# SeanChenxy/TDRN

Hardware: AMD Instinct MI355X
Metric: frames/sec/GPU @320x320 dualrefinedet_vggbn; box Linf vs CPU ref (higher is better)
Workload: dtype bf16; 1 GPU; dualrefinedet_vggbn 320x320 multihead, bf16, batch 32 per GPU, forward + Detect(top_k 200, conf 0.01, nms 0.45), synthetic VOC-shaped frames + synthetic weights; global_batch=32, parallelism=frame-sharded x1, no per-frame collective, launch=eager, resident_batches=4, steps_in_flight=2

## Files before the change

include/tdrn_hip.h:

```cpp
#ifndef TDRN_HIP_H
#define TDRN_HIP_H

#include <stddef.h>
#include <stdint.h>

#ifdef __cplusplus
extern "C" {
#endif

#define TDRN_API __attribute__((visibility("default")))

#define TDRN_OK 0
#define TDRN_E_ARG (-1)
#define TDRN_E_SHAPE (-2)
#define TDRN_E_WORKSPACE (-3)
#define TDRN_E_UNSUPPORTED (-4)
#define TDRN_E_PARAM (-5)
#define TDRN_E_STATE (-6)
#define TDRN_E_VALUE (-7)
#define TDRN_E_DEVICE (-8)

TDRN_API const char *tdrn_version(void);
TDRN_API const char *tdrn_error_string(int code);

// ... 161 lines not shown
#define TDRN_PLAN_ONE_STREAM    4
#define TDRN_PLAN_NO_DEFORM_TS  8
#define TDRN_PLAN_CHAIN         16
#define TDRN_PLAN_NO_CONV_PP    32
#define TDRN_PLAN_NO_PP_SK      64
#define TDRN_PLAN_NO_CONV_PATCH 128
#define TDRN_PLAN_DWPW          512
#define TDRN_PLAN_NO_PW1X1      1024
#define TDRN_PLAN_NO_DW_SLIDE   2048
#define TDRN_PLAN_DW_SLIDE_ALL  4096
#define TDRN_PLAN_NO_CONV_WS    8192
#define TDRN_PLAN_NO_YGEMM_V2  16384
#define TDRN_PLAN_NO_HEAD3X3   32768
#define TDRN_PLAN_TS_ONE_RANGE  65536
#define TDRN_PLAN_NO_PATCH_TAIL 131072
#define TDRN_PLAN_FAULT_HANDOFF 256

typedef struct tdrn_net tdrn_net;

TDRN_API int tdrn_net_create(const tdrn_net_config *cfg, tdrn_net **out);
TDRN_API void tdrn_net_destroy(tdrn_net *net);

TDRN_API int tdrn_net_param_count(const tdrn_net *net);
TDRN_API int tdrn_net_param_info(const tdrn_net *net, int index, const char **name,
                                 int64_t shape[4], int *ndim);
TDRN_API int tdrn_net_set_param(tdrn_net *net, const char *name, const float *data_host,
                                int64_t numel);

TDRN_API size_t tdrn_net_weight_bytes(const tdrn_net *net);
TDRN_API size_t tdrn_net_workspace_bytes(const tdrn_net *net, int batch);
// ... 72 lines not shown
```

tdrn_amd/_lib.py:

```python
import ctypes as C
import os

_HERE = os.path.dirname(os.path.abspath(__file__))
LIB_PATH = os.environ.get("TDRN_LIB_PATH") or os.path.join(_HERE, "lib", "libtdrn_hip.so")

F32, BF16, F16 = 0, 1, 2
DTYPES = {"fp32": F32, "f32": F32, "float32": F32, "bf16": BF16, "bfloat16": BF16, "fp16": F16,
          "f16": F16, "float16": F16, "half": F16}
DRN_VGGBN, DRN_MOBILENET, SSD4SCALE_MOBILE, REFINEDET_VGG, SSD4SCALE_VGG = range(5)

E_VALUE = -7


class TdrnError(RuntimeError):
    def __init__(self, code, what=""):
        self.code = code
        super().__init__("%s (tdrn error %d)%s" % (error_string(code), code,
                                                    (": " + what) if what else ""))


class NetConfig(C.Structure):
    _fields_ = [("model", C.c_int), ("size", C.c_int), ("num_classes", C.c_int),
                ("c7_channel", C.c_int), ("def_groups", C.c_int), ("bn", C.c_int),
                ("multihead", C.c_int), ("deform", C.c_int), ("test_phase", C.c_int),
                ("dtype", C.c_int), ("use_refine", C.c_int), ("plan_flags", C.c_int), ("reserved", C.c_int * 4)]


PLAN_NO_FUSE_FIRST, PLAN_NO_LATE_SIDE, PLAN_ONE_STREAM, PLAN_NO_DEFORM_TS, PLAN_CHAIN = 1, 2, 4, 8, 16
PLAN_NO_CONV_PP, PLAN_NO_PP_SK, PLAN_NO_CONV_PATCH, PLAN_FAULT_HANDOFF, PLAN_DWPW, PLAN_NO_PW1X1 = 32, 64, 128, 256, 512, 1024
PLAN_NO_DW_SLIDE, PLAN_DW_SLIDE_ALL, PLAN_NO_CONV_WS, PLAN_NO_YGEMM_V2, PLAN_NO_HEAD3X3, PLAN_TS_ONE_RANGE = 2048, 4096, 8192, 16384, 32768, 65536
PLAN_NO_PATCH_TAIL = 131072
E_DEVICE = -8


class NetIO(C.Structure):
    _fields_ = [("x", C.c_void_p), ("batch", C.c_int), ("arm_loc", C.c_void_p),
                ("odm_loc", C.c_void_p), ("conf", C.c_void_p), ("offsets", C.c_void_p * 4),
                ("ref_loc", C.c_void_p * 4), ("loc_maps", C.c_void_p * 4),
                ("reserved", C.c_void_p * 4)]


class KernelStat(C.Structure):
    _fields_ = [("name", C.c_char * 48), ("launches", C.c_int), ("flops", C.c_double),
                ("bytes", C.c_double), ("ms", C.c_double)]


# ... 166 lines not shown
```

tdrn_amd/csrc/conv3x3_patch.hip:

```cpp
#include <cstdio>
#include <cstdlib>
#include <type_traits>

#include "kernels.h"

#ifndef TDRN_PATCH_PRIO
#define TDRN_PATCH_PRIO 4
#endif
#ifndef TDRN_PATCH_ABLATE
#define TDRN_PATCH_ABLATE 0
#endif

namespace tdrn {

struct PatchParams {
    const char *in, *w, *zero;
    const float *bias;
    char *out, *out_pool;
    int B, H, W, Cin, Cout, Cs, Ktot;
    int relu;
    int tw, lgtw;
    int tiles_x, tiles_per_img;
    int m_tiles, n_tiles, items;
    int M;
    int tail_split;
    const float *fx, *fw, *fb;
    int fS, fCout;
    int ablate;
#ifdef TDRN_PATCH_STAMP
    unsigned *stamps;
#endif
#ifdef TDRN_PATCH_WGTIME
    unsigned long long *wgt;
#endif
};

#ifdef TDRN_PATCH_STAMP
#define STAMP_DECL unsigned long long st_t = __builtin_amdgcn_s_memtime(); unsigned st_acc[8] = {0, 0, 0, 0, 0, 0, 0, 0};
#define STAMP(k) do { const unsigned long long t_ = __builtin_amdgcn_s_memtime(); st_acc[k] += (unsigned)(t_ - st_t); st_t = t_; } while (0)
#define STAMP_FLUSH do { if (lane == 0) for (int k_ = 0; k_ < 8; ++k_) p.stamps[((size_t)blockIdx.x * 12 + wave) * 8 + k_] = st_acc[k_]; } while (0)
#else
#define STAMP_DECL
#define STAMP(k) do { } while (0)
// ... 76 lines not shown
    constexpr int RING = BN == 128 ? kRing : 3;
    constexpr int SROWS = (ES == 2 ? 16 : 8) / ((RING == 4 && BN == 128) ? 2 : 1);
    constexpr int SSTRIDE = BNH * ES + 16;
    constexpr int NPB = FUSE ? 1 : 2;
    constexpr int PSLOTS = FUSE ? ((TH + 2) * (TW + 2) + 7) / 8 : kPatchSlots;
    constexpr int PBYTES = PSLOTS * 1024;
    constexpr int OFF_W = NPB * PBYTES;
    constexpr int OFF_S = OFF_W + RING * WBYTES;
    constexpr int OFF_B = OFF_S + 8 * SROWS * SSTRIDE;
    constexpr int RAWR = TH + 4, RAWC = 36;
    constexpr int RAWN = 3 * RAWR * RAWC;
    constexpr int RAWP = (RAWN + 63) / 64, RAWJ = (RAWP + 3) / 4;
    constexpr int FTILES = ((TH + 2) * (TW + 2) + 31) / 32, FTJ = (FTILES + 3) / 4;
    constexpr int RAWB = ((RAWN + 63) / 64) * 256;
    constexpr int OFF_R = OFF_B + 1024;
    constexpr int LDS = FUSE ? OFF_R + 2 * RAWB + 256 : OFF_B + 1024;
    static_assert(LDS <= 160 * 1024, "LDS budget");
    __shared__ __attribute__((aligned(16))) char smem[LDS];

    const int lane = threadIdx.x & 63;
    const int wave = __builtin_amdgcn_readfirstlane(threadIdx.x >> 6);
    const int nchunks = p.Cin / CK;
#ifdef TDRN_PATCH_WGTIME
    if (threadIdx.x == 0) p.wgt[2 * blockIdx.x] = __builtin_amdgcn_s_memrealtime();
#endif

    const int xcd = blockIdx.x & 7, slot = blockIdx.x >> 3;
    const int per_xcd = (p.items + 7) >> 3, istride = ((int)gridDim.x + 7) >> 3;
    int avail = p.items - xcd * per_xcd;
    avail = avail < per_xcd ? avail : per_xcd;
    int n_full = avail > slot ? (avail - slot + istride - 1) / istride : 0;
    const int item0 = xcd * per_xcd + slot;
    [[maybe_unused]] int n_tail = 0, tail_enc = 0;
    constexpr bool TAILOK = BN == 128 && sizeof(DT) == 2 && !FUSE;
    if constexpr (TAILOK) {
        if (p.tail_split && avail > 0) {
            const int full = avail / istride, rem = avail - full * istride;
            if (full > 0 && rem > 0 && 2 * rem <= istride) {
                n_full = full;
                if (slot < 2 * rem) {
                    n_tail = 1;
                    tail_enc = 2 * (xcd * per_xcd + full * istride) + slot;
                }
            }
        }
    }
    const int n_it = n_full + n_tail;
    const int n_steps = n_it * nchunks * 9;
    auto item_mt = [&](int it) { return (it < n_full ? item0 + it * istride : tail_enc >> 1) / p.n_tiles; };
    auto item_c0 = [&](int it) {
        const int item = it < n_full ? item0 + it * istride : tail_enc >> 1;
        return (item % p.n_tiles) * BN + (it < n_full ? 0 : (tail_enc & 1) * 64);
    };
    const int RS = TW ? TW + 2 : p.W;

    if (wave >= 8) {
        if (TDRN_PATCH_PRIO == 4) __builtin_amdgcn_s_setprio(2);
        if (TDRN_PATCH_PRIO == 5) __builtin_amdgcn_s_setprio(3);
        const int lw = wave - 8;
        const int lrow = lane >> 3, pc = lane & 7;
        unsigned poff[kSlotsPerLoader];
        int pyx[kSlotsPerLoader];
        int plc[kSlotsPerLoader];
        {
#pragma unroll
            for (int j = 0; j < kSlotsPerLoader; ++j) {
                const int pr = (lw + 4 * j) * 8 + lrow;
                plc[j] = (pc ^ ((pr >> 1) & 7)) << 4;
// ... 131 lines not shown
#pragma unroll
                for (int j = 0; j < kSlotsPerLoader; ++j) {
                    const long long pix = j0 + pyx[j];
                    const bool ok = pyx[j] >= 0 && pix >= 0 && pix < p.M;
                    poff[j] = ok ? (unsigned)(pix * rowbytes + plc[j]) : 0xFFFFFFFFu;
                }
            }
        };
        unsigned woff[WL];
#pragma unroll
        for (int k = 0; k < WL; ++k) {
            const int n = (lw + 4 * k) * 8 + lrow;
            woff[k] = (unsigned)((size_t)n * p.Ktot * ES + ((pc ^ ((n >> 1) & 7)) << 4));
        }
        constexpr bool live = !(TDRN_PATCH_ABLATE & 1);
        int ws = 0, w_it = 0, w_cc = 0, w_tap = 0, wslot = 0;
        const char *wbase = p.w;
        unsigned wk = 0;
        int w_pieces = WL;
        auto weight_item = [&]() {
            wbase = p.w + (size_t)item_c0(w_it) * p.Ktot * ES;
            if constexpr (TAILOK) w_pieces = w_it < n_full ? WL : WL / 2;
        };
        constexpr bool wfixed = (TDRN_PATCH_ABLATE & 16) != 0, pfixed = (TDRN_PATCH_ABLATE & 32) != 0;
        auto load_weights = [&]() -> int {
            const int np = w_pieces;
            if (live) {
                char *dst = smem + OFF_W + wslot * WBYTES;
#pragma unroll
                for (int k = 0; k < WL; ++k)
                    if (!TAILOK || k < np) glds(wfixed ? p.w + (woff[k] & 0xffffu) : wbase + wk + woff[k], dst + (lw + 4 * k) * 1024);
            }
            ++ws;
            wslot = wslot == RING - 1 ? 0 : wslot + 1;
            wk += (unsigned)(p.Cin * ES);
            if (++w_tap == 9) {
                w_tap = 0;
                if (++w_cc == nchunks) {
                    w_cc = 0;
                    ++w_it;
                    if (w_it < n_it) weight_item();
                }
                wk = (unsigned)(w_cc * 128);
            }
            return np;
        };
        auto load_patch = [&](int j, unsigned ccoff, char *dstbuf) {
            if (!live || lw + 4 * j >= kPatchSlots || FUSE) return;
            const unsigned o = poff[j];
            glds(o == 0xFFFFFFFFu ? p.zero : (pfixed ? p.in + (o & 0xfffffu) : p.in + (size_t)o + ccoff), dstbuf + (lw + 4 * j) * 1024);
        };
        int p_it = 0, p_cc = 0, pbuf = 0;
        auto next_patch_chunk = [&]() {
            if (NPB == 2) pbuf ^= 1;
            if (++p_cc == nchunks) {
                p_cc = 0;
                ++p_it;
            }
        };

        if constexpr (FUSE) {
            if (n_it > 0) load_raw(item0, 0);
            asm volatile("s_waitcnt vmcnt(0) lgkmcnt(0)" ::: "memory");
            __builtin_amdgcn_s_barrier();
            if (n_it > 0) {
                int b_;
                tile_origin(item0, b_, f_y0, f_x0);
#pragma unroll
                for (int q = 0; q < FTJ; ++q)
                    if (lw + 4 * q < FTILES) first_conv_tile(lw + 4 * q, 0, smem);
            }
        }
        if (n_it > 0) {
            weight_item();
            if constexpr (!FUSE) {
                patch_table(item_mt(0));
#pragma unroll
                for (int j = 0; j < kSlotsPerLoader; ++j) load_patch(j, 0u, smem);
            }
#pragma unroll
            for (int k = 0; k < RING - 1; ++k)
                if (k < n_steps) load_weights();
            next_patch_chunk();
            if (lw == 0 && live)
                glds(lane < (n_full > 0 ? BN : 64) / 4 ? (const char *)(p.bias + item_c0(0)) + lane * 16 : p.zero, smem + OFF_B);
        }
        asm volatile("s_waitcnt vmcnt(0) lgkmcnt(0)" ::: "memory");
        __builtin_amdgcn_s_barrier();

        int tap = 0, c_it = 0, c_cc = 0, carried = 0;
        STAMP_DECL
        const int last_piece = lw + 4 * (kSlotsPerLoader - 1) < kPatchSlots ? 1 : 0;
        for (int g = 0; g < n_steps; ++g) {
            int issued = 0;
            if (ws < n_steps) issued = load_weights();
            if constexpr (FUSE) {
                if (tap == 0 && c_it + 1 < n_it) issued += load_raw(item0 + (c_it + 1) * istride, (c_it + 1) & 1);
            } else if (p_it < n_it && tap < 6) {
                char *dstbuf = smem + pbuf * PBYTES;
                const unsigned ccoff = (unsigned)(p_cc * 128);
                switch (tap) {
                    case 0:
                        patch_table(item_mt(p_it));
                        load_patch(0, ccoff, dstbuf); load_patch(1, ccoff, dstbuf); issued += 2; break;
                    case 1: load_patch(2, ccoff, dstbuf); load_patch(3, ccoff, dstbuf); issued += 2; break;
                    case 2: load_patch(4, ccoff, dstbuf); load_patch(5, ccoff, dstbuf); issued += 2; break;
                    case 3: load_patch(6, ccoff, dstbuf); load_patch(7, ccoff, dstbuf); issued += 2; break;
                    case 4: load_patch(8, ccoff, dstbuf); load_patch(9, ccoff, dstbuf); issued += 2; break;
                    default: load_patch(10, ccoff, dstbuf); issued += last_piece; break;
                }
            }
            if (lw == 0 && c_cc == nchunks - 1 && tap == 6 && c_it + 1 < n_it) {
                if (live) glds(lane < (c_it + 1 < n_full ? BN : 64) / 4 ? (const char *)(p.bias + item_c0(c_it + 1)) + lane * 16 : p.zero, smem + OFF_B);
                issued += 1;
            }
            STAMP(0);
            wait_vmcnt(live ? issued + (RING == 4 ? carried : 0) : 0);
            if constexpr (FUSE) asm volatile("s_waitcnt lgkmcnt(0)" ::: "memory");
            STAMP(1);
            carried = issued;
            __builtin_amdgcn_s_barrier();
            STAMP(2);
            if (++tap == 9) {
                tap = 0;
                next_patch_chunk();
                if (++c_cc == nchunks) {
                    if constexpr (FUSE) {
                        if (c_it + 1 < n_it) {
                            int b_;
                            tile_origin(item0 + (c_it + 1) * istride, b_, f_y0, f_x0);
#pragma unroll
                            for (int q = 0; q < FTJ; ++q)
                                if (lw + 4 * q < FTILES) first_conv_tile(lw + 4 * q, (c_it + 1) & 1, smem);
                            asm volatile("s_waitcnt lgkmcnt(0)" ::: "memory");
                            __builtin_amdgcn_s_barrier();
                        }
                    }
                    c_cc = 0;
                    ++c_it;
                }
            }
        }
        STAMP_FLUSH;
        return;
    }

    const int r32 = lane & 31, hh = lane >> 5;
    const int cw = wave % PXG;
    const int chalf = wave / PXG;
    char *stg = smem + OFF_S + wave * SROWS * SSTRIDE;
    f32x16 acc[WC][2];

    int base_i[2];
    unsigned tapmask[2] = {0x1FFu, 0x1FFu};
    unsigned need_mask = 0;
#pragma unroll
    for (int pt = 0; pt < 2; ++pt) {
        const int i = cw * 64 + pt * 32 + r32;
        base_i[pt] = TW ? (i >> LGTW) * RS + (i & (TW - 1)) : i;
    }
    const int wsw = (r32 >> 1) & 7;
    constexpr int CPR = BNH * ES / 16;
    constexpr int RPI = 64 / CPR;
    const int my_ch = lane % CPR, my_row = lane / CPR;
    constexpr bool compute = !(TDRN_PATCH_ABLATE & 2);

    int cur_mt = -1, n0 = 0;
    long long tile_pix0 = 0;
    int tile_row0 = 0, tile_x0 = 0;
    auto setup_item = [&](int it) {
        const int mt = item_mt(it);
        n0 = item_c0(it);
        if (mt == cur_mt) return;
        cur_mt = mt;
        if (TW) {
            const int b = mt / p.tiles_per_img, tt = mt - b * p.tiles_per_img;
            const int ty = tt / p.tiles_x, tx = tt - ty * p.tiles_x;
            tile_row0 = b * p.H + ty * TH;
            tile_x0 = tx * TW;
            tile_pix0 = (long long)tile_row0 * p.W + tile_x0;
            return;
        }
        tile_pix0 = (long long)mt * 256;
        need_mask = 0;
#pragma unroll
        for (int pt = 0; pt < 2; ++pt) {
            const long long m = tile_pix0 + cw * 64 + pt * 32 + r32;
// ... 230 lines not shown
    auto init_acc = [&](auto wcn_tag) {
        constexpr int WCN = decltype(wcn_tag)::value;
        const char *bsrc = smem + OFF_B;
#pragma unroll
        for (int ci = 0; ci < WCN; ++ci)
#pragma unroll
            for (int g = 0; g < 4; ++g) {
                const f32x4 bv = *(const f32x4 *)(bsrc + (chalf * (32 * WCN) + ci * 32 + 8 * g + 4 * hh) * 4);
#pragma unroll
                for (int pt = 0; pt < 2; ++pt)
#pragma unroll
                    for (int j = 0; j < 4; ++j) acc[ci][pt][4 * g + j] = bv[j];
            }
    };

    if constexpr (FUSE) __builtin_amdgcn_s_barrier();
    __builtin_amdgcn_s_barrier();
    if (TDRN_PATCH_PRIO == 2 && wave >= 4) __builtin_amdgcn_s_setprio(1);
    if (TDRN_PATCH_PRIO == 3) __builtin_amdgcn_s_setprio(1);
    typedef std::integral_constant<int, WC> full_t;
    typedef std::integral_constant<int, 1> half_t;
    if (n_it > 0) {
        setup_item(0);
        init_acc(full_t{});
        load_frags(full_t{}, wfA, pfA, 0);
    }
    int it = 0, cc = 0, tap = 0, tq = 0, delta = 0, wslot = 0, pbuf = 0;
    STAMP_DECL
    auto step = [&](auto wcn) {
        unsigned m0 = 0xFFFFFFFFu, m1 = 0xFFFFFFFFu;
        if constexpr (FLAT) {
            m0 = ((tapmask[0] >> tap) & 1u) ? 0xFFFFFFFFu : 0u;
            m1 = ((tapmask[1] >> tap) & 1u) ? 0xFFFFFFFFu : 0u;
        }
        if (TDRN_PATCH_PRIO == 0) __builtin_amdgcn_s_setprio(1);
        load_frags(wcn, wfB, pfB, 1);
        __builtin_amdgcn_sched_barrier(0);
        mma_frags(wcn, wfA, pfA, m0, m1);
        __builtin_amdgcn_sched_barrier(0);
        load_frags(wcn, wfA, pfA, 2);
        __builtin_amdgcn_sched_barrier(0);
        mma_frags(wcn, wfB, pfB, m0, m1);
// ... 21 lines not shown
        wsb = smem + OFF_W + wslot * WBYTES;
        psb = smem + (NPB == 2 ? pbuf : 0) * PBYTES;
#pragma unroll
        for (int pt = 0; pt < 2; ++pt) {
            prow[pt] = base_i[pt] + delta + tq;
            psw[pt] = (prow[pt] >> 1) & 7;
        }
        if (!(FUSE && item_done)) load_frags(wcn, wfA, pfA, 0);
        __builtin_amdgcn_sched_barrier(0);
        if (TDRN_PATCH_PRIO == 0) __builtin_amdgcn_s_setprio(1);
        mma_frags(wcn, wfB, pfB, m0, m1);
        if (TDRN_PATCH_PRIO == 0) __builtin_amdgcn_s_setprio(0);
        STAMP(2);
        if (item_done) {
            epilogue(wcn);
            ++it;
            if (it < n_it) {
                setup_item(it);
                if (TAILOK && it >= n_full) {
                    init_acc(half_t{});
                    load_frags(half_t{}, wfA, pfA, 0);
                } else {
                    init_acc(full_t{});
                }
                if constexpr (FUSE) {
                    __builtin_amdgcn_s_barrier();
                    load_frags(wcn, wfA, pfA, 0);
                }
            }
            STAMP(3);
        }
    };
    const int n_steps_full = n_full * nchunks * 9;
#pragma unroll 1
    for (int g = 0; g < n_steps_full; ++g) step(full_t{});
    if constexpr (TAILOK) {
#pragma unroll 1
        for (int g = n_steps_full; g < n_steps; ++g) step(half_t{});
    }
    STAMP_FLUSH;
#ifdef TDRN_PATCH_WGTIME
    if (threadIdx.x == 0) p.wgt[2 * blockIdx.x + 1] = __builtin_amdgcn_s_memrealtime();
#endif
}

int patch_conv_supported(const ConvArgs &a)
{
    if (a.kdisable & 4) return 0;
    if (a.kh != 3 || a.kw != 3 || a.stride != 1 || a.pad != 1 || a.dil != 1) return 0;
    if (a.phases != 1 || a.out_f32 || a.res) return 0;
    if (a.Ho != a.H || a.Wo != a.W) return 0;
    if (a.Npad % 64) return 0;
    if (a.o_rs != (long long)a.Wo * a.o_cs || a.o_bs != (long long)a.Ho * a.Wo * a.o_cs || a.o_base) return 0;
    if (!a.fuse_x && (long long)a.B * a.H * a.W * a.Cin * dtype_bytes(a.dtype) >= (1ll << 32)) return 0;
    if (a.W % 32 == 0 && a.H % 8 == 0) return 32;
    if (a.W % 16 == 0 && a.H % 16 == 0) return 16;
    if (2 * a.W + 2 + 256 <= kPatchSlots * 8) return -1;
    return 0;
}

template <typename DT, int BN> static int launch_patch_cfg(const PatchParams &p_in, hipStream_t s)
{
    PatchParams p = p_in;
    const int grid = p.items >= 256 ? 256 : ((p.items + 7) / 8) * 8;
#ifdef TDRN_PATCH_WGTIME
    static unsigned long long *wgt = nullptr;
    static long calls = 0, want = -1;
    if (!wgt) TDRN_HIP_TRY(hipMalloc((void **)&wgt, 256 * 2 * sizeof(unsigned long long)));
    if (want < 0) { const char *e = getenv("TDRN_WGTIME_CALL"); want = e ? atol(e) : 2000; }
    p.wgt = wgt;
    const bool report = calls >= want && calls < want + 18;
    ++calls;
    if (report) TDRN_HIP_TRY(hipMemsetAsync(wgt, 0, 256 * 2 * sizeof(unsigned long long), s));
    struct Report {
        bool on; hipStream_t s; int grid; const PatchParams &p; unsigned long long *d;
        ~Report() {
            if (!on) return;
            (void)hipStreamSynchronize(s);
            unsigned long long h[512];
            (void)hipMemcpy(h, d, sizeof(h), hipMemcpyDeviceToHost);
            unsigned long long t0 = ~0ull, t1 = 0;
            int n = 0;
            for (int i = 0; i < grid; ++i) if (h[2 * i]) { t0 = h[2 * i] < t0 ? h[2 * i] : t0; t1 = h[2 * i + 1] > t1 ? h[2 * i + 1] : t1; ++n; }
            double late = 0, busy = 0, worst = 0, e_min = 1e18; int n5 = 0, n20 = 0;
            for (int i = 0; i < grid; ++i) if (h[2 * i]) {
                const double d0 = (h[2 * i] - t0) * 0.01, b = (h[2 * i + 1] - h[2 * i]) * 0.01, e = (h[2 * i + 1] - t0) * 0.01;
                late += d0; busy += b; worst = d0 > worst ? d0 : worst; e_min = e < e_min ? e : e_min; n5 += d0 > 5; n20 += d0 > 20;
            }
            fprintf(stderr, "wgtime %dx%d Cin %d Cout %d items %d grid %d: span %.1f us, workgroup busy mean %.1f us, first end at %.1f us; start later than the first: mean %.1f us, max %.1f us, > 5 us: %d, > 20 us: %d of %d\n",
                    p.H, p.W, p.Cin, p.Cout, p.items, grid, (t1 - t0) * 0.01, busy / n, e_min, late / n, worst, n5, n20, n);
        }
    } rep{report, s, grid, p, wgt};
#endif
    if constexpr (BN == 64 && sizeof(DT) == 2) {
        if (p.fx) {
            if (p.tw != 32 || p.n_tiles != 1 || p.H % 16) return TDRN_E_UNSUPPORTED;
            hipLaunchKernelGGL((conv3x3_patch_kernel<DT, 64, 32, true>), dim3(grid), dim3(768), 0, s, p);
            return hip_status(hipGetLastError());
        }
    }
    if (p.fx) return TDRN_E_UNSUPPORTED;
    if (p.tw == 0) hipLaunchKernelGGL((conv3x3_patch_kernel<DT, BN, 0>), dim3(grid), dim3(768), 0, s, p);
    else if (p.tw == 32) hipLaunchKernelGGL((conv3x3_patch_kernel<DT, BN, 32>), dim3(grid), dim3(768), 0, s, p);
    else hipLaunchKernelGGL((conv3x3_patch_kernel<DT, BN, 16>), dim3(grid), dim3(768), 0, s, p);
    return hip_status(hipGetLastError());
// ... 25 lines not shown
        p.tiles_per_img = p.tiles_x * (a.H / ((a.fuse_x ? 512 : 256) / p.tw));
        p.m_tiles = a.B * p.tiles_per_img;
    } else {
        p.tiles_x = 0; p.tiles_per_img = 0;
        p.m_tiles = cdiv(p.M, 256);
    }
    int BN = a.Npad % 128 == 0 ? 128 : 64;
    if (BN == 128 && p.m_tiles * (a.Npad / 128) < 160) BN = 64;
    p.n_tiles = a.Npad / BN;
    p.items = p.m_tiles * p.n_tiles;
    static int ablate = -1;
    if (ablate < 0) ablate = dev_ablate_env("TDRN_CONV_ABLATE");
    p.ablate = ablate;
    p.fx = a.fuse_x; p.fw = a.fuse_w; p.fb = a.fuse_b; p.fS = a.H; p.fCout = a.fuse_cout;
    p.tail_split = !(a.kdisable & 1024);
    if (p.items <= 0) return TDRN_OK;
#ifdef TDRN_PATCH_STAMP
    static unsigned *stamps = nullptr;
    if (!stamps) TDRN_HIP_TRY(hipMalloc((void **)&stamps, 256 * 12 * 8 * sizeof(unsigned)));
    TDRN_HIP_TRY(hipMemsetAsync(stamps, 0, 256 * 12 * 8 * sizeof(unsigned), s));
    p.stamps = stamps;
    struct Report {
        const PatchParams &p; hipStream_t s; int BN, nchunks;
        ~Report()
        {
            static unsigned host[256 * 12 * 8];
            (void)hipStreamSynchronize(s);
            (void)hipMemcpy(host, p.stamps, sizeof(host), hipMemcpyDeviceToHost);
            double c[4] = {0, 0, 0, 0}, l[3] = {0, 0, 0};
            int nc = 0, nl = 0;
// ... 28 lines not shown
```

tdrn_amd/csrc/kernels.h:

```cpp
#pragma once
#include <cmath>

#include "common.h"

namespace tdrn {

constexpr size_t kZeroPageBytes = 256;

int allow_big_lds(const void *kernel);

struct ConvArgs {
    const void *in = nullptr, *w = nullptr, *res = nullptr, *zero_page = nullptr;
    const float *bias = nullptr;
    void *out = nullptr;
    int B = 0, H = 0, W = 0, Cin = 0;
    int Ho = 0, Wo = 0, Cout = 0, Npad = 0;
    int kh = 1, kw = 1, stride = 1, pad = 0, dil = 1;
    int relu = 0, out_f32 = 0, phases = 1;
    int splitk = 1;
    void *partial = nullptr;
    long long o_bs = 0, o_rs = 0, o_cs = 0, o_base = 0, o_pr = 0, o_pc = 0;
    int dtype = TDRN_BF16;
    const float *fuse_x = nullptr, *fuse_w = nullptr, *fuse_b = nullptr;
    int fuse_cout = 0;
    const unsigned char *fuse_x8 = nullptr;
    float fuse_mean[3] = {0.f, 0.f, 0.f};
    void *sk_ws = nullptr;
    bool sk_flags_zero = false;
    int kdisable = 0;
    unsigned *status = nullptr;
    int fault_handoff = 0;
};
int launch_conv(const ConvArgs &a, hipStream_t s);
struct ChainLayer { ConvArgs a; int dep[2] = {-1, -1}; };
int conv_chain_supported(const ConvArgs &a);
int conv_chain_max_layers();
size_t conv_chain_ctr_bytes();
int launch_conv_chain(const ChainLayer *layers, int n, unsigned *ctr, hipStream_t s, unsigned *status = nullptr);
int conv_splitk_choice(const ConvArgs &a);
size_t conv_splitk_bytes(const ConvArgs &a, int splits);
int head3x3_supported(const ConvArgs &a);
int launch_head3x3(const ConvArgs &a, hipStream_t s);
int patch_conv_supported(const ConvArgs &a);
// ... 142 lines not shown
```

tdrn_amd/csrc/net.hip:

```cpp
#include <algorithm>
#include <cmath>
#include <cstdlib>
#include <cstring>
#include <map>
#include <string>
#include <mutex>
#include <vector>

#include "kernels.h"

namespace tdrn {

unsigned short host_f32_to_bf16(float f)
{
    uint32_t u;
    memcpy(&u, &f, 4);
    if ((u & 0x7fffffffu) > 0x7f800000u) return (unsigned short)((u >> 16) | 0x40);
    return (unsigned short)((u + 0x7fffu + ((u >> 16) & 1u)) >> 16);
}
unsigned short host_f32_to_f16(float f)
{
    _Float16 h = (_Float16)f;
    unsigned short r;
    memcpy(&r, &h, 2);
// ... 106 lines not shown
    std::vector<ParamSpec> params;
    std::map<std::string, size_t> param_index;
    std::map<std::string, std::vector<float>> staged;
    std::vector<Op> ops;
    size_t ws_per_sample = 0, blob_bytes = kZeroPageBytes;
    size_t ws_fixed = 0;
    int P = 0, fm[4] = {0, 0, 0, 0}, scale_off[5] = {0, 0, 0, 0, 0};
    bool weights_ready = false;
    int profile = 0;
    std::vector<hipEvent_t> ev;
    std::vector<int> ev_stat;
    std::vector<int> ev_op;
    tdrn_kernel_stat stats[ST_COUNT];
    int last_batch = 0;
    static constexpr int kLanes = 4;
    static constexpr size_t kTailCtl = 256;
    size_t splitk_off[kLanes] = {0, 0, 0, 0};
    int cur_lane = 0;
    int t_late = -1;
    std::vector<int> chain_ops;
    size_t chain_partial_off = 0;
    bool pp_sk_planned = false;
    int fuse_first = -1;
    int x_t = -1;
    bool late_side = true;
    bool use_lanes = true, lanes_ready = false;
    bool y_tap_major = true;
    int plan_error = TDRN_OK;
    const void *offs_ws = nullptr;
    int offs_batch = 0, offs_key_batch = 0;
    int dev = -1;
// ... 454 lines not shown
            conv(src[s], "arm_conf." + ss, true, "", nc3, 3, 1, 1, 1, 0, -1, OUT_CONF, s);
            loc_maps_out(s);
        }
        if (cfg.test_phase) softmax_op();
        return TDRN_OK;
    }

    int build()
    {
        es = dtype_bytes(cfg.dtype);
        kdisable = ((cfg.plan_flags & TDRN_PLAN_NO_CONV_PP) ? 1 : 0) | ((cfg.plan_flags & TDRN_PLAN_NO_PP_SK) ? 2 : 0) |
                   ((cfg.plan_flags & TDRN_PLAN_NO_CONV_PATCH) ? 4 : 0) | ((cfg.plan_flags & TDRN_PLAN_NO_PW1X1) ? 8 : 0) |
                   ((cfg.plan_flags & TDRN_PLAN_NO_DW_SLIDE) ? 16 : 0) | ((cfg.plan_flags & TDRN_PLAN_DW_SLIDE_ALL) ? 32 : 0) |
                   ((cfg.plan_flags & TDRN_PLAN_NO_CONV_WS) ? 64 : 0) | ((cfg.plan_flags & TDRN_PLAN_NO_YGEMM_V2) ? 128 : 0) |
                   ((cfg.plan_flags & TDRN_PLAN_NO_HEAD3X3) ? 256 : 0) | ((cfg.plan_flags & TDRN_PLAN_TS_ONE_RANGE) ? 512 : 0) |
                   ((cfg.plan_flags & TDRN_PLAN_NO_PATCH_TAIL) ? 1024 : 0);
        fault_handoff = (cfg.plan_flags & TDRN_PLAN_FAULT_HANDOFF) ? 1 : 0;
        if (cfg.size < 128 || cfg.size > 1280 || cfg.size % 64 != 0) return TDRN_E_ARG;
        if (cfg.num_classes < 2 || cfg.num_classes > 21 * 4) return TDRN_E_ARG;
        if (cfg.dtype < 0 || cfg.dtype > 2) return TDRN_E_ARG;
        if (cfg.def_groups < 1) return TDRN_E_ARG;
        int rc;
        switch (cfg.model) {
            case TDRN_DRN_VGGBN: rc = build_drn_vgg(); break;
            case TDRN_DRN_MOBILENET: rc = build_drn_mobilenet(); break;
            case TDRN_SSD4SCALE_MOBILE: rc = build_ssd4scale(true); break;
            case TDRN_SSD4SCALE_VGG: rc = build_ssd4scale(false); break;
            case TDRN_REFINEDET_VGG: rc = build_refinedet_vgg(); break;
            default: return TDRN_E_UNSUPPORTED;
        }
        if (rc != TDRN_OK) return rc;
// ... 153 lines not shown
                DwPwArgs a;
                a.B = 1; a.H = ti.H; a.W = ti.W; a.Cin = c.Cin; a.Cout = c.Cout; a.Npad = c.Npad; a.Cs = tensors[c.out].Cpad;
                a.stride = d.stride; a.dtype = cfg.dtype;
                if (ti.Cpad != c.Cin || !dwpw_supported(a)) continue;
                d.fused_dw = 1; c.fused_dw = 1;
                d.stat = ST_DWPW;
                d.flops += c.flops;
                d.bytes = (double)ti.H * ti.W * ti.Cpad * es + (double)ti.H * ti.W * tensors[c.out].Cpad * es;
                c.flops = 0; c.bytes = 0;
            }
        ws_fixed = 0;
        pp_sk_planned = false;
        if (cfg.dtype != TDRN_F32)
            for (const Op &o : ops)
                if (o.kind == OP_CONV && o.stat == ST_CONV3 && o.lane == 0 && o.Cin >= 256 && o.Npad % 256 == 0) pp_sk_planned = true;
        if (pp_sk_planned || !chain_ops.empty()) ws_fixed = kTailCtl + (pp_sk_planned ? align_up(conv_pp_sk_bytes(), 256) : 1024);
        use_lanes = !(cfg.plan_flags & TDRN_PLAN_ONE_STREAM);
        y_tap_major = true;
        for (const Op &d : ops)
            if (d.kind == OP_DEFORM && d.y_t >= 0 && !ygemm_supported(d.Cin, d.y_cols, cfg.dtype)) y_tap_major = false;
        tensor_lane.assign(tensors.size(), 0);
        tensor_shared.assign(tensors.size(), 0);
        for (const Op &o : ops) {
            if (o.out >= 0) tensor_lane[o.out] = o.lane;
            if (o.pool_t >= 0) tensor_lane[o.pool_t] = o.lane;
        }
        for (const Op &o : ops)
            for (int t : {o.in, o.res, o.off_t})
                if (t >= 0 && tensor_lane[t] != o.lane) tensor_shared[t] = 1;
        return TDRN_OK;
    }
// ... 271 lines not shown
                    if ((ops[k].n_branches == 2 || (ops[k].G >= 2 && ops[k].G % 2 == 0)) && ops[k].y_t < 0 && !dsplit) dsplit = &ops[k];
                    if (k == 0 || ops[k - 1].kind != OP_DEFORM) ++n_deform_groups;
                }
            if (dsplit && n_deform_groups == 1) {
                float *locbase0 = dsplit->out_kind == OUT_ARM_LOC ? io->arm_loc : io->odm_loc;
                TDRN_HIP_TRY(hipStreamWaitEvent(side[0], ev_fork, 0));
                lane_used[1] = true;
                TDRN_HIP_TRY(hipMemsetAsync(locbase0, 0, (size_t)B * P * 4 * sizeof(float), side[0]));
                TDRN_HIP_TRY(hipMemsetAsync(io->conf, 0, (size_t)B * P * C * sizeof(float), side[0]));
                TDRN_HIP_TRY(hipEventRecord(ev_zero, side[0]));
                zeroed_early = true;
            }
        }
        bool skz_pending = false;
        char *const tail = (char *)ws + ws_per_sample * (size_t)B;
        if (ws_fixed) {
            if (lanes) {
                if (!lane_used[1]) {
                    TDRN_HIP_TRY(hipStreamWaitEvent(side[0], ev_fork, 0));
                    lane_used[1] = true;
                }
                TDRN_HIP_TRY(hipMemsetAsync(tail, 0, kTailCtl + 1024, side[0]));
                TDRN_HIP_TRY(hipEventRecord(ev_skz, side[0]));
                skz_pending = true;
            } else {
                TDRN_HIP_TRY(hipMemsetAsync(tail, 0, kTailCtl + 1024, s0));
            }
        }
        auto conv_args = [&](const Op &o, ConvArgs &a) {
            const Tensor &ti = tensors[o.in];
            a.in = tptr(ws, o.in, B); a.w = wb + o.w_off; a.bias = (const float *)(wb + o.b_off); a.zero_page = wb;
            a.B = B; a.H = ti.H; a.W = ti.W; a.Cin = o.Cin; a.Ho = o.hw >> 16; a.Wo = o.hw & 0xffff;
            a.Cout = o.Cout; a.Npad = o.Npad; a.kh = a.kw = o.k; a.stride = o.stride; a.pad = o.pad; a.dil = o.dil;
            a.relu = o.relu; a.phases = o.phases; a.dtype = cfg.dtype;
            a.kdisable = kdisable; a.status = status; a.fault_handoff = fault_handoff;
            if (o.out_kind == OUT_TENSOR) {
                const Tensor &to = tensors[o.out];
                a.out = tptr(ws, o.out, B);
                if (o.res >= 0) a.res = tptr(ws, o.res, B);
                a.o_cs = to.Cpad;
                if (o.phases == 4) {
                    a.o_bs = (long long)to.H * to.W * to.Cpad; a.o_rs = 2ll * to.W * to.Cpad; a.o_cs = 2ll * to.Cpad;
                    a.o_pr = (long long)to.W * to.Cpad; a.o_pc = to.Cpad;
                } else {
                    a.o_bs = (long long)to.H * to.W * to.Cpad; a.o_rs = (long long)to.W * to.Cpad;
                }
            } else {
                const int per = o.out_kind == OUT_CONF ? 3 * C : 12;
                const int per_prior = o.out_kind == OUT_CONF ? C : 4;
                float *base = o.out_kind == OUT_ARM_LOC ? io->arm_loc : (o.out_kind == OUT_ODM_LOC ? io->odm_loc : io->conf);
// ... 82 lines not shown
                        }
                        if (skz_pending) {
                            TDRN_HIP_TRY(hipStreamWaitEvent(s0, ev_skz, 0));
                            skz_pending = false;
                        }
                        rc = launch_conv_chain(cl, n, (unsigned *)tail, s, status);
                        if (rc == TDRN_OK && lanes)
                            for (int k = 1; k < n; ++k) {
                                const int t = ops[chain_ops[k]].out;
                                if (t >= 0 && tensor_shared[t]) TDRN_HIP_TRY(hipEventRecord(tensor_ev[t], s));
                            }
                        break;
                    }
                    ConvArgs a;
                    conv_args(o, a);
                    if (o.lane == 0 && pp_sk_planned) {
                        a.sk_ws = tail + kTailCtl;
                        a.sk_flags_zero = true;
                        if (skz_pending && pp_conv_supported(a)) {
                            TDRN_HIP_TRY(hipStreamWaitEvent(s0, ev_skz, 0));
                            skz_pending = false;
                        }
                    }
                    if ((int)oi == fuse_first) {
                        a.fuse_w = (const float *)(wb + ops[0].w_off); a.fuse_b = (const float *)(wb + ops[0].b_off);
                        a.fuse_cout = ops[0].Cout;
                        if (!xin && o.pool_t >= 0) {
                            a.fuse_x8 = u8->planes; a.fuse_mean[0] = u8->mean[0]; a.fuse_mean[1] = u8->mean[1]; a.fuse_mean[2] = u8->mean[2];
                            a.out = nullptr;
                            rc = ws_conv_supported(a) ? launch_conv3x3_ws(a, tptr(ws, o.pool_t, B), s) : TDRN_E_UNSUPPORTED;
// ... 509 lines not shown
```

Baseline: 12510 frames/s.

## Replace static item dealing in patch conv with per-XCD atomic work claiming

The patch 3x3 conv kernel now has a loader wave claim work units dynamically through a per-XCD global atomic counter, instead of each workgroup taking a fixed strided set of items. The claimed unit, which can be a full tile or a half tail unit, is passed to the compute waves through a two-slot LDS mailbox. The last workgroup to finish resets the counters, and the host reserves per-lane claim slots in the workspace tail and waits on the zeroing event before first use. This is meant to even out load imbalance when workgroups start late, at the cost of atomic latency, an extra mailbox handshake in the pipeline, and new cross-stream ordering requirements.

```diff
diff --git a/include/tdrn_hip.h b/include/tdrn_hip.h
--- a/include/tdrn_hip.h
+++ b/include/tdrn_hip.h
@@ -199,6 +199,7 @@
 #define TDRN_PLAN_NO_HEAD3X3   32768
 #define TDRN_PLAN_TS_ONE_RANGE  65536
 #define TDRN_PLAN_NO_PATCH_TAIL 131072
+#define TDRN_PLAN_NO_PATCH_CLAIM 262144
 #define TDRN_PLAN_FAULT_HANDOFF 256
 
 typedef struct tdrn_net tdrn_net;
diff --git a/tdrn_amd/_lib.py b/tdrn_amd/_lib.py
--- a/tdrn_amd/_lib.py
+++ b/tdrn_amd/_lib.py
@@ -29,7 +29,7 @@
 PLAN_NO_FUSE_FIRST, PLAN_NO_LATE_SIDE, PLAN_ONE_STREAM, PLAN_NO_DEFORM_TS, PLAN_CHAIN = 1, 2, 4, 8, 16
 PLAN_NO_CONV_PP, PLAN_NO_PP_SK, PLAN_NO_CONV_PATCH, PLAN_FAULT_HANDOFF, PLAN_DWPW, PLAN_NO_PW1X1 = 32, 64, 128, 256, 512, 1024
 PLAN_NO_DW_SLIDE, PLAN_DW_SLIDE_ALL, PLAN_NO_CONV_WS, PLAN_NO_YGEMM_V2, PLAN_NO_HEAD3X3, PLAN_TS_ONE_RANGE = 2048, 4096, 8192, 16384, 32768, 65536
-PLAN_NO_PATCH_TAIL = 131072
+PLAN_NO_PATCH_TAIL, PLAN_NO_PATCH_CLAIM = 131072, 262144
 E_DEVICE = -8
 
 
diff --git a/tdrn_amd/csrc/conv3x3_patch.hip b/tdrn_amd/csrc/conv3x3_patch.hip
--- a/tdrn_amd/csrc/conv3x3_patch.hip
+++ b/tdrn_amd/csrc/conv3x3_patch.hip
@@ -27,6 +27,7 @@
     const float *fx, *fw, *fb;
     int fS, fCout;
     int ablate;
+    unsigned *claim;
 #ifdef TDRN_PATCH_STAMP
     unsigned *stamps;
 #endif
@@ -133,7 +134,8 @@
     constexpr int FTILES = ((TH + 2) * (TW + 2) + 31) / 32, FTJ = (FTILES + 3) / 4;
     constexpr int RAWB = ((RAWN + 63) / 64) * 256;
     constexpr int OFF_R = OFF_B + 1024;
-    constexpr int LDS = FUSE ? OFF_R + 2 * RAWB + 256 : OFF_B + 1024;
+    constexpr int OFF_M = FUSE ? OFF_R + 2 * RAWB + 256 : OFF_B + 1024;
+    constexpr int LDS = OFF_M + 16;
     static_assert(LDS <= 160 * 1024, "LDS budget");
     __shared__ __attribute__((aligned(16))) char smem[LDS];
 
@@ -141,36 +143,17 @@
     const int wave = __builtin_amdgcn_readfirstlane(threadIdx.x >> 6);
     const int nchunks = p.Cin / CK;
 #ifdef TDRN_PATCH_WGTIME
-    if (threadIdx.x == 0) p.wgt[2 * blockIdx.x] = __builtin_amdgcn_s_memrealtime();
+    if (threadIdx.x == 0) p.wgt[3 * blockIdx.x] = __builtin_amdgcn_s_memrealtime();
 #endif
 
     const int xcd = blockIdx.x & 7, slot = blockIdx.x >> 3;
     const int per_xcd = (p.items + 7) >> 3, istride = ((int)gridDim.x + 7) >> 3;
-    int avail = p.items - xcd * per_xcd;
-    avail = avail < per_xcd ? avail : per_xcd;
-    int n_full = avail > slot ? (avail - slot + istride - 1) / istride : 0;
-    const int item0 = xcd * per_xcd + slot;
-    [[maybe_unused]] int n_tail = 0, tail_enc = 0;
+    typedef volatile __attribute__((address_space(3))) int lds_int;
+    lds_int *const mbox = (lds_int *)(smem + OFF_M);
     constexpr bool TAILOK = BN == 128 && sizeof(DT) == 2 && !FUSE;
-    if constexpr (TAILOK) {
-        if (p.tail_split && avail > 0) {
-            const int full = avail / istride, rem = avail - full * istride;
-            if (full > 0 && rem > 0 && 2 * rem <= istride) {
-                n_full = full;
-                if (slot < 2 * rem) {
-                    n_tail = 1;
-                    tail_enc = 2 * (xcd * per_xcd + full * istride) + slot;
-                }
-            }
-        }
-    }
-    const int n_it = n_full + n_tail;
-    const int n_steps = n_it * nchunks * 9;
-    auto item_mt = [&](int it) { return (it < n_full ? item0 + it * istride : tail_enc >> 1) / p.n_tiles; };
-    auto item_c0 = [&](int it) {
-        const int item = it < n_full ? item0 + it * istride : tail_enc >> 1;
-        return (item % p.n_tiles) * BN + (it < n_full ? 0 : (tail_enc & 1) * 64);
-    };
+    auto unit_mt = [&](int u) { return (u >> 2) / p.n_tiles; };
+    auto unit_half = [&](int u) { return TAILOK && (u & 2) != 0; };
+    auto unit_c0 = [&](int u) { return ((u >> 2) % p.n_tiles) * BN + (unit_half(u) ? (u & 1) * 64 : 0); };
     const int RS = TW ? TW + 2 : p.W;
 
     if (wave >= 8) {
@@ -332,13 +315,50 @@
             woff[k] = (unsigned)((size_t)n * p.Ktot * ES + ((pc ^ ((n >> 1) & 7)) << 4));
         }
         constexpr bool live = !(TDRN_PATCH_ABLATE & 1);
-        int ws = 0, w_it = 0, w_cc = 0, w_tap = 0, wslot = 0;
+        int n_whole = p.items - xcd * per_xcd;
+        n_whole = n_whole < per_xcd ? n_whole : per_xcd;
+        n_whole = n_whole > 0 ? n_whole : 0;
+        int n_units = n_whole;
+        if constexpr (TAILOK) {
+            if (p.tail_split) {
+                const int full = n_whole / istride, rem = n_whole - full * istride;
+                if (full > 0 && rem > 0 && 2 * rem <= istride) {
+                    n_whole = full * istride;
+                    n_units = n_whole + 2 * rem;
+                }
+            }
+        }
+        auto unit_of = [&](int k) -> int {
+            const int h = k - n_whole, base = xcd * per_xcd;
+            return (unsigned)k >= (unsigned)n_units ? -1 : (h < 0 ? (base + k) << 2 : (((base + n_whole + (h >> 1)) << 2) | 2 | (h & 1)));
+        };
+        int k_pend = 0, k_dealt = slot - istride;
+        auto claim_issue = [&]() -> int {
+            if (p.claim) {
+                if (lane == 0) k_pend = (int)__hip_atomic_fetch_add(p.claim + xcd, 1u, __ATOMIC_RELAXED, __HIP_MEMORY_SCOPE_AGENT);
+                return 1;
+            }
+            k_dealt += istride;
+            return 0;
+        };
+        auto claim_publish = [&](int m) {
+            if (p.claim) {
+                if (lane == 0) mbox[m & 1] = unit_of(k_pend);
+            } else if (lane == 0) {
+                mbox[m & 1] = unit_of(k_dealt);
+            }
+        };
+        int w_cc = 0, w_tap = 0, wslot = 0;
+        bool w_live = false;
         const char *wbase = p.w;
         unsigned wk = 0;
         int w_pieces = WL;
-        auto weight_item = [&]() {
-            wbase = p.w + (size_t)item_c0(w_it) * p.Ktot * ES;
-            if constexpr (TAILOK) w_pieces = w_it < n_full ? WL : WL / 2;
+        int u_p = -1;
+        auto weight_item = [&](int u) {
+            w_live = u >= 0;
+            if (!w_live) return;
+            wbase = p.w + (size_t)unit_c0(u) * p.Ktot * ES;
+            if constexpr (TAILOK) w_pieces = unit_half(u) ? WL / 2 : WL;
         };
         constexpr bool wfixed = (TDRN_PATCH_ABLATE & 16) != 0, pfixed = (TDRN_PATCH_ABLATE & 32) != 0;
         auto load_weights = [&]() -> int {
@@ -349,15 +369,13 @@
                 for (int k = 0; k < WL; ++k)
                     if (!TAILOK || k < np) glds(wfixed ? p.w + (woff[k] & 0xffffu) : wbase + wk + woff[k], dst + (lw + 4 * k) * 1024);
             }
-            ++ws;
             wslot = wslot == RING - 1 ? 0 : wslot + 1;
             wk += (unsigned)(p.Cin * ES);
             if (++w_tap == 9) {
                 w_tap = 0;
                 if (++w_cc == nchunks) {
                     w_cc = 0;
-                    ++w_it;
-                    if (w_it < n_it) weight_item();
+                    weight_item(u_p);
                 }
                 wk = (unsigned)(w_cc * 128);
             }
@@ -377,49 +395,63 @@
             }
         };
 
+        if (lw == 0) {
+            claim_issue();
+            claim_publish(0);
+            if (nchunks == 1) {
+                claim_issue();
+                claim_publish(1);
+            }
+        }
+        asm volatile("s_waitcnt vmcnt(0) lgkmcnt(0)" ::: "memory");
+        __builtin_amdgcn_s_barrier();
+        int u_c = __builtin_amdgcn_readfirstlane(mbox[0]);
+        u_p = u_c;
         if constexpr (FUSE) {
-            if (n_it > 0) load_raw(item0, 0);
+            if (u_c >= 0) load_raw(u_c >> 2, 0);
             asm volatile("s_waitcnt vmcnt(0) lgkmcnt(0)" ::: "memory");
             __builtin_amdgcn_s_barrier();
-            if (n_it > 0) {
+            if (u_c >= 0) {
                 int b_;
-                tile_origin(item0, b_, f_y0, f_x0);
+                tile_origin(u_c >> 2, b_, f_y0, f_x0);
 #pragma unroll
                 for (int q = 0; q < FTJ; ++q)
                     if (lw + 4 * q < FTILES) first_conv_tile(lw + 4 * q, 0, smem);
             }
         }
-        if (n_it > 0) {
-            weight_item();
+        if (u_c >= 0) {
+            weight_item(u_c);
             if constexpr (!FUSE) {
-                patch_table(item_mt(0));
+                patch_table(unit_mt(u_c));
 #pragma unroll
                 for (int j = 0; j < kSlotsPerLoader; ++j) load_patch(j, 0u, smem);
             }
 #pragma unroll
-            for (int k = 0; k < RING - 1; ++k)
-                if (k < n_steps) load_weights();
+            for (int k = 0; k < RING - 1; ++k) load_weights();
             next_patch_chunk();
             if (lw == 0 && live)
-                glds(lane < (n_full > 0 ? BN : 64) / 4 ? (const char *)(p.bias + item_c0(0)) + lane * 16 : p.zero, smem + OFF_B);
+                glds(lane < (unit_half(u_c) ? 64 : BN) / 4 ? (const char *)(p.bias + unit_c0(u_c)) + lane * 16 : p.zero, smem + OFF_B);
         }
         asm volatile("s_waitcnt vmcnt(0) lgkmcnt(0)" ::: "memory");
         __builtin_amdgcn_s_barrier();
 
-        int tap = 0, c_it = 0, c_cc = 0, carried = 0;
+        int tap = 0, c_cc = 0, carried = 0;
+        [[maybe_unused]] int c_it = 0;
         STAMP_DECL
         const int last_piece = lw + 4 * (kSlotsPerLoader - 1) < kPatchSlots ? 1 : 0;
-        for (int g = 0; g < n_steps; ++g) {
+        while (u_c >= 0) {
             int issued = 0;
-            if (ws < n_steps) issued = load_weights();
+            if (tap == 0 && p_cc == 0) u_p = __builtin_amdgcn_readfirstlane(mbox[p_it & 1]);
+            if (lw == 0 && tap == 3 && p_cc == nchunks - 1 && u_p >= 0) claim_publish(p_it + 1);
+            if (w_live) issued = load_weights();
             if constexpr (FUSE) {
-                if (tap == 0 && c_it + 1 < n_it) issued += load_raw(item0 + (c_it + 1) * istride, (c_it + 1) & 1);
-            } else if (p_it < n_it && tap < 6) {
+                if (tap == 0 && c_cc == nchunks - 1 && u_p >= 0) issued += load_raw(u_p >> 2, (c_it + 1) & 1);
+            } else if (u_p >= 0 && tap < 6) {
                 char *dstbuf = smem + pbuf * PBYTES;
                 const unsigned ccoff = (unsigned)(p_cc * 128);
                 switch (tap) {
                     case 0:
-                        patch_table(item_mt(p_it));
+                        patch_table(unit_mt(u_p));
                         load_patch(0, ccoff, dstbuf); load_patch(1, ccoff, dstbuf); issued += 2; break;
                     case 1: load_patch(2, ccoff, dstbuf); load_patch(3, ccoff, dstbuf); issued += 2; break;
                     case 2: load_patch(4, ccoff, dstbuf); load_patch(5, ccoff, dstbuf); issued += 2; break;
@@ -428,13 +460,14 @@
                     default: load_patch(10, ccoff, dstbuf); issued += last_piece; break;
                 }
             }
-            if (lw == 0 && c_cc == nchunks - 1 && tap == 6 && c_it + 1 < n_it) {
-                if (live) glds(lane < (c_it + 1 < n_full ? BN : 64) / 4 ? (const char *)(p.bias + item_c0(c_it + 1)) + lane * 16 : p.zero, smem + OFF_B);
+            if (lw == 0 && c_cc == nchunks - 1 && tap == 6 && u_p >= 0) {
+                if (live) glds(lane < (unit_half(u_p) ? 64 : BN) / 4 ? (const char *)(p.bias + unit_c0(u_p)) + lane * 16 : p.zero, smem + OFF_B);
                 issued += 1;
             }
+            if (lw == 0 && tap == 1 && p_cc == nchunks - 1 && u_p >= 0) issued += claim_issue();
             STAMP(0);
             wait_vmcnt(live ? issued + (RING == 4 ? carried : 0) : 0);
-            if constexpr (FUSE) asm volatile("s_waitcnt lgkmcnt(0)" ::: "memory");
+            if (FUSE || (lw == 0 && tap == 3)) asm volatile("s_waitcnt lgkmcnt(0)" ::: "memory");
             STAMP(1);
             carried = issued;
             __builtin_amdgcn_s_barrier();
@@ -444,9 +477,9 @@
                 next_patch_chunk();
                 if (++c_cc == nchunks) {
                     if constexpr (FUSE) {
-                        if (c_it + 1 < n_it) {
+                        if (u_p >= 0) {
                             int b_;
-                            tile_origin(item0 + (c_it + 1) * istride, b_, f_y0, f_x0);
+                            tile_origin(u_p >> 2, b_, f_y0, f_x0);
 #pragma unroll
                             for (int q = 0; q < FTJ; ++q)
                                 if (lw + 4 * q < FTILES) first_conv_tile(lw + 4 * q, (c_it + 1) & 1, smem);
@@ -456,10 +489,16 @@
                     }
                     c_cc = 0;
                     ++c_it;
+                    u_c = u_p;
                 }
             }
         }
         STAMP_FLUSH;
+        if (lw == 0 && lane == 0 && p.claim) {
+            const unsigned done = __hip_atomic_fetch_add(p.claim + 8, 1u, __ATOMIC_RELAXED, __HIP_MEMORY_SCOPE_AGENT);
+            if (done == gridDim.x - 1)
+                for (int i = 0; i < 9; ++i) __hip_atomic_store(p.claim + i, 0u, __ATOMIC_RELAXED, __HIP_MEMORY_SCOPE_AGENT);
+        }
         return;
     }
 
@@ -486,9 +525,9 @@
     int cur_mt = -1, n0 = 0;
     long long tile_pix0 = 0;
     int tile_row0 = 0, tile_x0 = 0;
-    auto setup_item = [&](int it) {
-        const int mt = item_mt(it);
-        n0 = item_c0(it);
+    auto setup_item = [&](int u) {
+        const int mt = unit_mt(u);
+        n0 = unit_c0(u);
         if (mt == cur_mt) return;
         cur_mt = mt;
         if (TW) {
@@ -749,18 +788,26 @@
             }
     };
 
+    __builtin_amdgcn_s_barrier();
+    int u_cur = __builtin_amdgcn_readfirstlane(mbox[0]);
+    int n_done = 0;
     if constexpr (FUSE) __builtin_amdgcn_s_barrier();
     __builtin_amdgcn_s_barrier();
     if (TDRN_PATCH_PRIO == 2 && wave >= 4) __builtin_amdgcn_s_setprio(1);
     if (TDRN_PATCH_PRIO == 3) __builtin_amdgcn_s_setprio(1);
     typedef std::integral_constant<int, WC> full_t;
     typedef std::integral_constant<int, 1> half_t;
-    if (n_it > 0) {
-        setup_item(0);
-        init_acc(full_t{});
-        load_frags(full_t{}, wfA, pfA, 0);
-    }
-    int it = 0, cc = 0, tap = 0, tq = 0, delta = 0, wslot = 0, pbuf = 0;
+    if (u_cur >= 0) {
+        setup_item(u_cur);
+        if (unit_half(u_cur)) {
+            init_acc(half_t{});
+            load_frags(half_t{}, wfA, pfA, 0);
+        } else {
+            init_acc(full_t{});
+            load_frags(full_t{}, wfA, pfA, 0);
+        }
+    }
+    int cc = 0, tap = 0, tq = 0, delta = 0, wslot = 0, pbuf = 0;
     STAMP_DECL
     auto step = [&](auto wcn) {
         unsigned m0 = 0xFFFFFFFFu, m1 = 0xFFFFFFFFu;
@@ -812,10 +859,11 @@
         STAMP(2);
         if (item_done) {
             epilogue(wcn);
-            ++it;
-            if (it < n_it) {
-                setup_item(it);
-                if (TAILOK && it >= n_full) {
+            ++n_done;
+            u_cur = __builtin_amdgcn_readfirstlane(mbox[n_done & 1]);
+            if (u_cur >= 0) {
+                setup_item(u_cur);
+                if (unit_half(u_cur)) {
                     init_acc(half_t{});
                     load_frags(half_t{}, wfA, pfA, 0);
                 } else {
@@ -829,16 +877,18 @@
             STAMP(3);
         }
     };
-    const int n_steps_full = n_full * nchunks * 9;
 #pragma unroll 1
-    for (int g = 0; g < n_steps_full; ++g) step(full_t{});
+    while (u_cur >= 0 && !unit_half(u_cur)) step(full_t{});
     if constexpr (TAILOK) {
 #pragma unroll 1
-        for (int g = n_steps_full; g < n_steps; ++g) step(half_t{});
+        while (u_cur >= 0) step(half_t{});
     }
     STAMP_FLUSH;
 #ifdef TDRN_PATCH_WGTIME
-    if (threadIdx.x == 0) p.wgt[2 * blockIdx.x + 1] = __builtin_amdgcn_s_memrealtime();
+    if (threadIdx.x == 0) {
+        p.wgt[3 * blockIdx.x + 1] = __builtin_amdgcn_s_memrealtime();
+        p.wgt[3 * blockIdx.x + 2] = (unsigned long long)n_done;
+    }
 #endif
 }
 
@@ -864,29 +914,33 @@
 #ifdef TDRN_PATCH_WGTIME
     static unsigned long long *wgt = nullptr;
     static long calls = 0, want = -1;
-    if (!wgt) TDRN_HIP_TRY(hipMalloc((void **)&wgt, 256 * 2 * sizeof(unsigned long long)));
+    if (!wgt) TDRN_HIP_TRY(hipMalloc((void **)&wgt, 256 * 3 * sizeof(unsigned long long)));
     if (want < 0) { const char *e = getenv("TDRN_WGTIME_CALL"); want = e ? atol(e) : 2000; }
     p.wgt = wgt;
     const bool report = calls >= want && calls < want + 18;
     ++calls;
-    if (report) TDRN_HIP_TRY(hipMemsetAsync(wgt, 0, 256 * 2 * sizeof(unsigned long long), s));
+    if (report) TDRN_HIP_TRY(hipMemsetAsync(wgt, 0, 256 * 3 * sizeof(unsigned long long), s));
     struct Report {
         bool on; hipStream_t s; int grid; const PatchParams &p; unsigned long long *d;
         ~Report() {
             if (!on) return;
             (void)hipStreamSynchronize(s);
-            unsigned long long h[512];
+            unsigned long long h[768];
             (void)hipMemcpy(h, d, sizeof(h), hipMemcpyDeviceToHost);
             unsigned long long t0 = ~0ull, t1 = 0;
             int n = 0;
-            for (int i = 0; i < grid; ++i) if (h[2 * i]) { t0 = h[2 * i] < t0 ? h[2 * i] : t0; t1 = h[2 * i + 1] > t1 ? h[2 * i + 1] : t1; ++n; }
+            for (int i = 0; i < grid; ++i) if (h[3 * i]) { t0 = h[3 * i] < t0 ? h[3 * i] : t0; t1 = h[3 * i + 1] > t1 ? h[3 * i + 1] : t1; ++n; }
             double late = 0, busy = 0, worst = 0, e_min = 1e18; int n5 = 0, n20 = 0;
-            for (int i = 0; i < grid; ++i) if (h[2 * i]) {
-                const double d0 = (h[2 * i] - t0) * 0.01, b = (h[2 * i + 1] - h[2 * i]) * 0.01, e = (h[2 * i + 1] - t0) * 0.01;
+            double u_sum = 0, u_early = 0, u_late = 0; int u_min = 1 << 30, u_max = 0;
+            for (int i = 0; i < grid; ++i) if (h[3 * i]) {
+                const double d0 = (h[3 * i] - t0) * 0.01, b = (h[3 * i + 1] - h[3 * i]) * 0.01, e = (h[3 * i + 1] - t0) * 0.01;
                 late += d0; busy += b; worst = d0 > worst ? d0 : worst; e_min = e < e_min ? e : e_min; n5 += d0 > 5; n20 += d0 > 20;
-            }
-            fprintf(stderr, "wgtime %dx%d Cin %d Cout %d items %d grid %d: span %.1f us, workgroup busy mean %.1f us, first end at %.1f us; start later than the first: mean %.1f us, max %.1f us, > 5 us: %d, > 20 us: %d of %d\n",
-                    p.H, p.W, p.Cin, p.Cout, p.items, grid, (t1 - t0) * 0.01, busy / n, e_min, late / n, worst, n5, n20, n);
+                const int u = (int)h[3 * i + 2];
+                u_sum += u; (d0 > 5 ? u_late : u_early) += u; u_min = u < u_min ? u : u_min; u_max = u > u_max ? u : u_max;
+            }
+            fprintf(stderr, "wgtime %dx%d Cin %d Cout %d items %d grid %d: span %.1f us, workgroup busy mean %.1f us, first end at %.1f us; start later than the first: mean %.1f us, max %.1f us, > 5 us: %d, > 20 us: %d of %d; units per workgroup min %d mean %.2f max %d (%s; started within 5 us: mean %.2f, later: mean %.2f)\n",
+                    p.H, p.W, p.Cin, p.Cout, p.items, grid, (t1 - t0) * 0.01, busy / n, e_min, late / n, worst, n5, n20, n,
+                    u_min, u_sum / n, u_max, p.claim ? "claimed" : "dealt", n - n5 ? u_early / (n - n5) : 0.0, n5 ? u_late / n5 : 0.0);
         }
     } rep{report, s, grid, p, wgt};
 #endif
@@ -942,6 +996,7 @@
     p.ablate = ablate;
     p.fx = a.fuse_x; p.fw = a.fuse_w; p.fb = a.fuse_b; p.fS = a.H; p.fCout = a.fuse_cout;
     p.tail_split = !(a.kdisable & 1024);
+    p.claim = ((a.kdisable & 2048) || a.fuse_x) ? nullptr : (unsigned *)a.patch_claim;
     if (p.items <= 0) return TDRN_OK;
 #ifdef TDRN_PATCH_STAMP
     static unsigned *stamps = nullptr;
diff --git a/tdrn_amd/csrc/kernels.h b/tdrn_amd/csrc/kernels.h
--- a/tdrn_amd/csrc/kernels.h
+++ b/tdrn_amd/csrc/kernels.h
@@ -27,6 +27,7 @@
     float fuse_mean[3] = {0.f, 0.f, 0.f};
     void *sk_ws = nullptr;
     bool sk_flags_zero = false;
+    void *patch_claim = nullptr;
     int kdisable = 0;
     unsigned *status = nullptr;
     int fault_handoff = 0;
diff --git a/tdrn_amd/csrc/net.hip b/tdrn_amd/csrc/net.hip
--- a/tdrn_amd/csrc/net.hip
+++ b/tdrn_amd/csrc/net.hip
@@ -144,7 +144,7 @@
     tdrn_kernel_stat stats[ST_COUNT];
     int last_batch = 0;
     static constexpr int kLanes = 4;
-    static constexpr size_t kTailCtl = 256;
+    static constexpr size_t kTailClaim = 256, kTailCtl = kTailClaim + 64 * kLanes;
     size_t splitk_off[kLanes] = {0, 0, 0, 0};
     int cur_lane = 0;
     int t_late = -1;
@@ -629,7 +629,7 @@
                    ((cfg.plan_flags & TDRN_PLAN_NO_DW_SLIDE) ? 16 : 0) | ((cfg.plan_flags & TDRN_PLAN_DW_SLIDE_ALL) ? 32 : 0) |
                    ((cfg.plan_flags & TDRN_PLAN_NO_CONV_WS) ? 64 : 0) | ((cfg.plan_flags & TDRN_PLAN_NO_YGEMM_V2) ? 128 : 0) |
                    ((cfg.plan_flags & TDRN_PLAN_NO_HEAD3X3) ? 256 : 0) | ((cfg.plan_flags & TDRN_PLAN_TS_ONE_RANGE) ? 512 : 0) |
-                   ((cfg.plan_flags & TDRN_PLAN_NO_PATCH_TAIL) ? 1024 : 0);
+                   ((cfg.plan_flags & TDRN_PLAN_NO_PATCH_TAIL) ? 1024 : 0) | ((cfg.plan_flags & TDRN_PLAN_NO_PATCH_CLAIM) ? 2048 : 0);
         fault_handoff = (cfg.plan_flags & TDRN_PLAN_FAULT_HANDOFF) ? 1 : 0;
         if (cfg.size < 128 || cfg.size > 1280 || cfg.size % 64 != 0) return TDRN_E_ARG;
         if (cfg.num_classes < 2 || cfg.num_classes > 21 * 4) return TDRN_E_ARG;
@@ -813,7 +813,7 @@
         if (cfg.dtype != TDRN_F32)
             for (const Op &o : ops)
                 if (o.kind == OP_CONV && o.stat == ST_CONV3 && o.lane == 0 && o.Cin >= 256 && o.Npad % 256 == 0) pp_sk_planned = true;
-        if (pp_sk_planned || !chain_ops.empty()) ws_fixed = kTailCtl + (pp_sk_planned ? align_up(conv_pp_sk_bytes(), 256) : 1024);
+        if (cfg.dtype != TDRN_F32 || !chain_ops.empty()) ws_fixed = kTailCtl + (pp_sk_planned ? align_up(conv_pp_sk_bytes(), 256) : 1024);
         use_lanes = !(cfg.plan_flags & TDRN_PLAN_ONE_STREAM);
         y_tap_major = true;
         for (const Op &d : ops)
@@ -1115,6 +1115,7 @@
         }
         bool skz_pending = false;
         char *const tail = (char *)ws + ws_per_sample * (size_t)B;
+        bool ctl_zero_seen[kLanes] = {false, true, false, false};
         if (ws_fixed) {
             if (lanes) {
                 if (!lane_used[1]) {
@@ -1135,6 +1136,7 @@
             a.Cout = o.Cout; a.Npad = o.Npad; a.kh = a.kw = o.k; a.stride = o.stride; a.pad = o.pad; a.dil = o.dil;
             a.relu = o.relu; a.phases = o.phases; a.dtype = cfg.dtype;
             a.kdisable = kdisable; a.status = status; a.fault_handoff = fault_handoff;
+            a.patch_claim = ws_fixed ? tail + kTailClaim + 64 * (lanes ? o.lane : 0) : nullptr;
             if (o.out_kind == OUT_TENSOR) {
                 const Tensor &to = tensors[o.out];
                 a.out = tptr(ws, o.out, B);
@@ -1247,6 +1249,11 @@
                     }
                     ConvArgs a;
                     conv_args(o, a);
+                    if (lanes && a.patch_claim && !(kdisable & 2048) && !ctl_zero_seen[lane] && patch_conv_supported(a)) {
+                        TDRN_HIP_TRY(hipStreamWaitEvent(s, ev_skz, 0));
+                        ctl_zero_seen[lane] = true;
+                        if (lane == 0) skz_pending = false;
+                    }
                     if (o.lane == 0 && pp_sk_planned) {
                         a.sk_ws = tail + kTailCtl;
                         a.sk_flags_zero = true;
```

New measurement: 11880 frames/s. 0.949x the previous value.
